# Research-Implementation/AudioVidSum-A-Multi-Modal-Approach-to-Video-Summarization

Hardware: AMD Instinct MI355X
Metric: frames/sec end-to-end (extract+fuse+score), 224x224 + 16kHz (higher is better)
Workload: dtype f16x2; 1 GPU; configs[1]: SumMe-shape batch, 25 videos x ~1800 frames (45143 frames/GPU), visual-only resnet50 extractor (batch-stat BN, the reference's 4-frame BatchNorm micro-batches inside each video) + AVBiLSTM attention scorer + mean-threshold selection; frames_per_gpu=45143, videos_per_gpu=25, extractor=resnet50, frames_per_group=4, chunk_frames=16384, parallelism=videos sharded x1, no data-path collective, selected_frames_rank0=22823

## Files before the change

audiovidsum-a-multi-modal-approach-to-video-summarization_amd/csrc/stem_h2.hip:

```cpp
#include "avs_internal.h"
#include <type_traits>

typedef _Float16 f16x8 __attribute__((ext_vector_type(8)));
typedef float f32x16 __attribute__((ext_vector_type(16)));

namespace {
constexpr int IMG = 224, CONV = 112, POOL = 56, COUT = 64;
constexpr int TY = 7, TX = 8;
constexpr int TH = 17, TWD = 15;
constexpr int PPY = 8, PPX = 7;
constexpr int MROWS = TH * TWD;
constexpr int PH = 39, PW = 36;
constexpr int PATCH_BYTES = PH * PW * 8;
constexpr int KDIM = 224;
constexpr int CW = 32;
constexpr int W_PITCH = KDIM * 4 + 16;
constexpr int W_BYTES = CW * W_PITCH;
constexpr int RT_PITCH = 144;
constexpr int RT_BYTES = 256 * RT_PITCH;
constexpr int WAVES = 4, THREADS = WAVES * 64;
constexpr int SRED_BYTES = WAVES * 2 * CW * 4, PIV_BYTES = CW * 4;
constexpr int SMEM_BYTES = W_BYTES + PATCH_BYTES + RT_BYTES + SRED_BYTES + PIV_BYTES;
constexpr int PIVOT_ROW = 9 * TWD + 7;
static_assert(SMEM_BYTES <= 80 * 1024, "two workgroups per CU");
}

struct StemH2Params {
  const uint8_t* frames;
  const char* w;
  const float* gamma;
  char* osel;
  float* part;
  long long ldw;
};

struct __attribute__((packed, aligned(1))) avs_u32_unaligned { unsigned v; };

__global__ __launch_bounds__(THREADS, 2) void stem_h2_kernel(StemH2Params p) {
  extern __shared__ __attribute__((aligned(16))) char smem[];
  char* wimg = smem;
  char* patch = smem + W_BYTES;
  char* rawt = patch + PATCH_BYTES;
  float* sred = reinterpret_cast<float*>(rawt + RT_BYTES);
  float* piv_s = sred + WAVES * 2 * CW;
  const int t = threadIdx.x;
  const int wave = __builtin_amdgcn_readfirstlane(t >> 6), lane = t & 63;
  const int lr = lane & 31, lh = lane >> 5;
  const int c0 = (blockIdx.x & 1) * CW;
  const long long img = blockIdx.x >> 1;
  const uint8_t* __restrict__ src = p.frames + img * (long long)(IMG * IMG * 3);

  for (int i = t; i < CW * (KDIM / 4); i += THREADS) {
    const int n = i / (KDIM / 4), ch = i - n * (KDIM / 4);
    *reinterpret_cast<uint4*>(wimg + n * W_PITCH + ch * 16) =
        *reinterpret_cast<const uint4*>(p.w + ((long long)(c0 + n) * p.ldw) * 4 + ch * 16);
  }
  int abase[2];
  unsigned own = 0;
#pragma unroll
  for (int mt = 0; mt < 2; ++mt) {
    int m = wave * 64 + mt * 32 + lr;
    if (m >= MROWS) m = MROWS - 1;
    const int ly = m / TWD, lx = m - ly * TWD;
    abase[mt] = ((2 * ly) * PW + 2 * lx) * 8 + lh * 16;
#pragma unroll
    for (int e = 0; e < 16; ++e) {
      const int me = wave * 64 + mt * 32 + (e & 3) + 8 * (e >> 2) + 4 * lh;
      const int ey = me / TWD, ex = me - ey * TWD;
      if (me < MROWS && ey >= 1 && ex >= 1) own |= 1u << (16 * mt + e);
    }
  }
  const int bbase = lr * W_PITCH + lh * 32;
  const bool pool_on = t < PPY * PPX * 4;
  const int p_cg = t & 3, p_pp = pool_on ? (t >> 2) : 0;
  const int p_pyl = p_pp / PPX, p_pxl = p_pp - p_pyl * PPX;
  float sg[8];
#pragma unroll
  for (int j = 0; j < 8; ++j) sg[j] = p.gamma[c0 + p_cg * 8 + j] < 0.f ? -1.f : 1.f;
  const char* praw = rawt + ((2 * p_pyl) * TWD + 2 * p_pxl) * RT_PITCH + p_cg * 32;

  constexpr int PPT = (PH * PW + THREADS - 1) / THREADS;
  unsigned pbytes[PPT];
  unsigned inside = 0u;
  int pyx[PPT];
#pragma unroll
  for (int j = 0; j < PPT; ++j) {
    const int i = t + j * THREADS;
    const int py = i < PH * PW ? i / PW : 255;
    pyx[j] = (py << 8) | (i - (i / PW) * PW);
  }
  auto gload = [&](int tile) {
    const int ty = tile / TX, tx = tile - ty * TX;
    const int iy0 = 32 * ty - 5, ix0 = 28 * tx - 5;
    const int ylo = iy0 < 0 ? -iy0 : 0, yhi = IMG - iy0 < PH ? IMG - iy0 : PH;
    const int xlo = ix0 < 0 ? -ix0 : 0, xhi = IMG - ix0 < PW ? IMG - ix0 : PW;
    inside = 0u;
#pragma unroll
    for (int j = 0; j < PPT; ++j) {
      const int py = pyx[j] >> 8, px = pyx[j] & 255;
      if (py >= ylo && py < yhi && px >= xlo && px < xhi) {
        const int o = ((iy0 + py) * IMG + ix0 + px) * 3;
        const bool prev = o > 0 || img > 0;
        const unsigned d = reinterpret_cast<const avs_u32_unaligned*>(src + o - (prev ? 1 : 0))->v;
        pbytes[j] = prev ? d >> 8 : d;
        inside |= 1u << j;
      }
    }
  };
  auto pstore = [&]() {
#pragma unroll
    for (int j = 0; j < PPT; ++j) {
      const int i = t + j * THREADS;
      if (i >= PH * PW) break;
      unsigned lo = 0u, hi = 0u;
      if ((inside >> j) & 1u) {
        const float b0 = (float)(pbytes[j] & 255u), b1 = (float)((pbytes[j] >> 8) & 255u), b2 = (float)((pbytes[j] >> 16) & 255u);
        lo = __builtin_bit_cast(unsigned, __builtin_amdgcn_cvt_pkrtz(b0, b1));
        hi = __builtin_bit_cast(unsigned, __builtin_amdgcn_cvt_pkrtz(b2, 1.f));
      }
      *reinterpret_cast<uint2*>(patch + i * 8) = make_uint2(lo, hi);
    }
  };
  float pm[8];
  auto pool_tap = [&](int tile, int tap) {
    const int ty = tile / TX, tx = tile - ty * TX;
    const int dy = tap / 3, dx = tap - dy * 3;
    const bool out = (dy == 0 && ty == 0 && p_pyl == 0) || (dx == 0 && tx == 0 && p_pxl == 0);
    const char* row = praw + (dy * TWD + dx) * RT_PITCH;
    const float4 va = *reinterpret_cast<const float4*>(row);
    const float4 vb = *reinterpret_cast<const float4*>(row + 16);
    const float v[8] = {va.x, va.y, va.z, va.w, vb.x, vb.y, vb.z, vb.w};
#pragma unroll
    for (int j = 0; j < 8; ++j) {
      float x = v[j] * sg[j];
      if (dy == 0 || dx == 0) x = out ? -INFINITY : x;
      pm[j] = tap == 0 ? x : fmaxf(pm[j], x);
    }
  };
  auto pool_finish = [&](int tile) {
    const int ty = tile / TX, tx = tile - ty * TX;
    float v8[8];
#pragma unroll
    for (int j = 0; j < 8; ++j) v8[j] = pm[j] * sg[j];
    uint4 hi, lo;
    avs_f16x2_split8(v8, hi, lo);
    const long long o = (((img * POOL + PPY * ty + p_pyl) * POOL + PPX * tx + p_pxl) * COUT + c0 + p_cg * 8) * 4;
    if (pool_on) {
      *reinterpret_cast<uint4*>(p.osel + o) = hi;
      *reinterpret_cast<uint4*>(p.osel + o + 16) = lo;
    }
  };

  gload(0);
  float pivot = 0.f, s1 = 0.f, s2 = 0.f;
  constexpr int NT = TY * TX;
  auto body = [&](auto pool_c, int tile) {
    constexpr bool POOLING = decltype(pool_c)::value;
    pstore();
    __syncthreads();
    if (tile + 1 < NT) gload(tile + 1);

    f32x16 acc[2];
#pragma unroll
    for (int i = 0; i < 2; ++i)
#pragma unroll
      for (int e = 0; e < 16; ++e) acc[i][e] = 0.f;
#pragma unroll
    for (int s = 0; s < 14; ++s) {
      const int aoff = (s >> 1) * (PW * 8) + (s & 1) * 32;
      uint4 fa[2];
#pragma unroll
      for (int mt = 0; mt < 2; ++mt) fa[mt] = *reinterpret_cast<const uint4*>(patch + abase[mt] + aoff);
      const uint4 fbh = *reinterpret_cast<const uint4*>(wimg + bbase + s * 64);
      const uint4 fbl = *reinterpret_cast<const uint4*>(wimg + bbase + s * 64 + 16);
#pragma unroll
      for (int mt = 0; mt < 2; ++mt)
        acc[mt] = __builtin_amdgcn_mfma_f32_32x32x16_f16(__builtin_bit_cast(f16x8, fa[mt]), __builtin_bit_cast(f16x8, fbh),
                                                         acc[mt], 0, 0, 0);
#pragma unroll
      for (int mt = 0; mt < 2; ++mt)
        acc[mt] = __builtin_amdgcn_mfma_f32_32x32x16_f16(__builtin_bit_cast(f16x8, fa[mt]), __builtin_bit_cast(f16x8, fbl),
                                                         acc[mt], 0, 0, 0);
      if constexpr (POOLING) {
        if (s < 9) pool_tap(tile - 1, s);
        if (s == 9) pool_finish(tile - 1);
      }
    }
    if (tile == 0 && wave == PIVOT_ROW / 64 && lh == ((PIVOT_ROW % 32) >> 2 & 1)) {
      constexpr int PMT = (PIVOT_ROW % 64) / 32, PR = PIVOT_ROW % 32;
      constexpr int PE = (PR & 3) + 4 * (PR >> 3);
      piv_s[lr] = acc[PMT][PE];
    }
    __syncthreads();
    if (tile == 0) pivot = piv_s[lr];
    float t1 = 0.f, t2 = 0.f;
#pragma unroll
    for (int mt = 0; mt < 2; ++mt)
#pragma unroll
      for (int e = 0; e < 16; ++e) {
        const float v = acc[mt][e];
        const float d = ((own >> (16 * mt + e)) & 1u) ? v - pivot : 0.f;
        t1 += d;
        t2 = fmaf(d, d, t2);
        const int m = wave * 64 + mt * 32 + (e & 3) + 8 * (e >> 2) + 4 * lh;
        *reinterpret_cast<float*>(rawt + m * RT_PITCH + lr * 4) = v;
      }
    s1 += t1;
    s2 += t2;
  };
  body(std::false_type{}, 0);
  for (int tile = 1; tile < NT; ++tile) body(std::true_type{}, tile);
  __syncthreads();
#pragma unroll
  for (int tap = 0; tap < 9; ++tap) pool_tap(NT - 1, tap);
  pool_finish(NT - 1);
  s1 += __shfl_xor(s1, 32, 64);
  s2 += __shfl_xor(s2, 32, 64);
  if (lh == 0) {
    sred[(wave * 2 + 0) * CW + lr] = s1;
    sred[(wave * 2 + 1) * CW + lr] = s2;
  }
  __syncthreads();
  if (t < CW) {
    float a = 0.f, b = 0.f;
#pragma unroll
    for (int w = 0; w < WAVES; ++w) {
      a += sred[(w * 2 + 0) * CW + t];
      b += sred[(w * 2 + 1) * CW + t];
    }
    const float inv_n = 1.f / (float)(CONV * CONV);
    const float dm = a * inv_n;
    p.part[(img * 2 + 0) * COUT + c0 + t] = piv_s[t] + dm;
    p.part[(img * 2 + 1) * COUT + c0 + t] = fmaxf(b - a * dm, 0.f);
  }
}

__global__ __launch_bounds__(256) void stem_h2_fold_kernel(const float* __restrict__ part, int groups, int fpg,
                                                           const float* __restrict__ gamma, const float* __restrict__ beta,
                                                           float eps, float* __restrict__ scale, float* __restrict__ shift) {
  const int i = blockIdx.x * blockDim.x + threadIdx.x;
  if (i >= groups * COUT) return;
  const int g = i / COUT, ch = i - g * COUT;
  const float nf = (float)(CONV * CONV);
  float n = 0.f, mean = 0.f, m2 = 0.f;
  for (int f = 0; f < fpg; ++f) {
    const long long fr = (long long)g * fpg + f;
    const float mf = part[(fr * 2 + 0) * COUT + ch], qf = part[(fr * 2 + 1) * COUT + ch];
    const float tot = n + nf, delta = mf - mean;
    mean += delta * (nf / tot);
    m2 += qf + delta * delta * (n * nf / tot);
    n = tot;
  }
  const float var = m2 / n;
  const float sc = gamma[ch] / sqrtf(var + eps);
  scale[i] = sc;
  shift[i] = beta[ch] - mean * sc;
}

extern "C" int64_t avs_stem_f16x2_workspace_bytes(int n) {
  if (n < 0) return AVS_E_SHAPE;
  return (int64_t)n * 2 * COUT * 4;
}

extern "C" int avs_stem_conv_pool_f16x2(const uint8_t* d_frames, int n, const void* d_w, int64_t ldw,
                                        int frames_per_group, const float* d_gamma, const float* d_beta, float eps,
                                        void* d_y, float* d_scale, float* d_shift, void* d_ws, int64_t ws_bytes,
                                        avs_stream_t stream) {
  const char* who = "avs_stem_conv_pool_f16x2";
  AVS_REQUIRE(n >= 0 && frames_per_group > 0, AVS_E_SHAPE, "%s: n=%d frames_per_group=%d", who, n, frames_per_group);
  if (n == 0) return AVS_OK;
  AVS_REQUIRE(n % frames_per_group == 0, AVS_E_UNSUPPORTED, "%s: needs equal-sized groups (%d frames in groups of %d)",
              who, n, frames_per_group);
  AVS_REQUIRE(d_frames && d_w && d_gamma && d_beta && d_y && d_scale && d_shift && d_ws, AVS_E_ARG,
              "%s: null pointer", who);
  AVS_REQUIRE(ldw >= KDIM && ldw % 8 == 0, AVS_E_SHAPE, "%s: weight rows are 7 x 8 x 4 = 224 slots, stride %lld", who,
              (long long)ldw);
  AVS_REQUIRE((((uintptr_t)d_w) & 31u) == 0 && (((uintptr_t)d_y) & 31u) == 0 && avs_aligned16(d_ws) &&
                  avs_aligned16(d_scale) && avs_aligned16(d_shift),
              AVS_E_ALIGN, "%s: AVS_F16X2 operands must be 32-byte aligned, the others 16-byte", who);
  const int64_t need = avs_stem_f16x2_workspace_bytes(n);
  AVS_REQUIRE(ws_bytes >= need, AVS_E_WORKSPACE, "%s: workspace %lld < %lld bytes", who, (long long)ws_bytes,
              (long long)need);
  AVS_REQUIRE((long long)n * 2 < (1ll << 31), AVS_E_SHAPE, "%s: too many frames", who);
  StemH2Params p{};
  p.frames = d_frames;
  p.w = (const char*)d_w;
  p.ldw = ldw;
  p.gamma = d_gamma;
  p.osel = (char*)d_y;
  p.part = reinterpret_cast<float*>(d_ws);
  hipStream_t st = (hipStream_t)stream;
  AVS_REQUIRE(hipFuncSetAttribute(reinterpret_cast<const void*>(stem_h2_kernel), hipFuncAttributeMaxDynamicSharedMemorySize,
                                  SMEM_BYTES) == hipSuccess,
              AVS_E_HIP, "%s: cannot reserve %d bytes of LDS", who, SMEM_BYTES);
  hipLaunchKernelGGL(stem_h2_kernel, dim3((unsigned)(n * 2)), dim3(THREADS), SMEM_BYTES, st, p);
  const int groups = n / frames_per_group;
  hipLaunchKernelGGL(stem_h2_fold_kernel, dim3((unsigned)avs_cdiv((int64_t)groups * COUT, 256)), dim3(256), 0, st, p.part,
                     groups, frames_per_group, d_gamma, d_beta, eps, d_scale, d_shift);
  AVS_CHECK_LAUNCH(who);
  return AVS_OK;
}
```

Measured before the change: 27160 frames/s.

## Hold stem conv weights in registers and double-buffer patch fragment loads

The stem conv kernel no longer stages the weight slice in LDS. Each lane instead loads its 14 K-steps of B fragments directly from global memory into registers, which frees LDS and removes the per-step LDS weight reads. The A-fragment LDS loads are software-pipelined one K-step ahead. The gather load is made branchless, with the byte-shift moved into pstore, and the pool_on guard on the output store is dropped. The cost is roughly 112 extra VGPRs per lane for the weights, which risks spills or lower occupancy under launch_bounds(256,2). Dropping the store guard may also let idle threads write duplicate or out-of-range pooled outputs.

```diff
diff --git a/audiovidsum-a-multi-modal-approach-to-video-summarization_amd/csrc/stem_h2.hip b/audiovidsum-a-multi-modal-approach-to-video-summarization_amd/csrc/stem_h2.hip
--- a/audiovidsum-a-multi-modal-approach-to-video-summarization_amd/csrc/stem_h2.hip
+++ b/audiovidsum-a-multi-modal-approach-to-video-summarization_amd/csrc/stem_h2.hip
@@ -14,13 +14,12 @@
 constexpr int PATCH_BYTES = PH * PW * 8;
 constexpr int KDIM = 224;
 constexpr int CW = 32;
-constexpr int W_PITCH = KDIM * 4 + 16;
-constexpr int W_BYTES = CW * W_PITCH;
+constexpr int KSTEPS = KDIM / 16;
 constexpr int RT_PITCH = 144;
 constexpr int RT_BYTES = 256 * RT_PITCH;
 constexpr int WAVES = 4, THREADS = WAVES * 64;
 constexpr int SRED_BYTES = WAVES * 2 * CW * 4, PIV_BYTES = CW * 4;
-constexpr int SMEM_BYTES = W_BYTES + PATCH_BYTES + RT_BYTES + SRED_BYTES + PIV_BYTES;
+constexpr int SMEM_BYTES = PATCH_BYTES + RT_BYTES + SRED_BYTES + PIV_BYTES;
 constexpr int PIVOT_ROW = 9 * TWD + 7;
 static_assert(SMEM_BYTES <= 80 * 1024, "two workgroups per CU");
 }
@@ -38,8 +37,7 @@
 
 __global__ __launch_bounds__(THREADS, 2) void stem_h2_kernel(StemH2Params p) {
   extern __shared__ __attribute__((aligned(16))) char smem[];
-  char* wimg = smem;
-  char* patch = smem + W_BYTES;
+  char* patch = smem;
   char* rawt = patch + PATCH_BYTES;
   float* sred = reinterpret_cast<float*>(rawt + RT_BYTES);
   float* piv_s = sred + WAVES * 2 * CW;
@@ -50,10 +48,14 @@
   const long long img = blockIdx.x >> 1;
   const uint8_t* __restrict__ src = p.frames + img * (long long)(IMG * IMG * 3);
 
-  for (int i = t; i < CW * (KDIM / 4); i += THREADS) {
-    const int n = i / (KDIM / 4), ch = i - n * (KDIM / 4);
-    *reinterpret_cast<uint4*>(wimg + n * W_PITCH + ch * 16) =
-        *reinterpret_cast<const uint4*>(p.w + ((long long)(c0 + n) * p.ldw) * 4 + ch * 16);
+  uint4 fbh[KSTEPS], fbl[KSTEPS];
+  {
+    const char* __restrict__ wrow = p.w + ((long long)(c0 + lr) * p.ldw) * 4 + lh * 32;
+#pragma unroll
+    for (int s = 0; s < KSTEPS; ++s) {
+      fbh[s] = *reinterpret_cast<const uint4*>(wrow + s * 64);
+      fbl[s] = *reinterpret_cast<const uint4*>(wrow + s * 64 + 16);
+    }
   }
   int abase[2];
   unsigned own = 0;
@@ -70,7 +72,6 @@
       if (me < MROWS && ey >= 1 && ex >= 1) own |= 1u << (16 * mt + e);
     }
   }
-  const int bbase = lr * W_PITCH + lh * 32;
   const bool pool_on = t < PPY * PPX * 4;
   const int p_cg = t & 3, p_pp = pool_on ? (t >> 2) : 0;
   const int p_pyl = p_pp / PPX, p_pxl = p_pp - p_pyl * PPX;
@@ -81,7 +82,7 @@
 
   constexpr int PPT = (PH * PW + THREADS - 1) / THREADS;
   unsigned pbytes[PPT];
-  unsigned inside = 0u;
+  unsigned inside = 0u, first = 0u;
   int pyx[PPT];
 #pragma unroll
   for (int j = 0; j < PPT; ++j) {
@@ -95,16 +96,16 @@
     const int ylo = iy0 < 0 ? -iy0 : 0, yhi = IMG - iy0 < PH ? IMG - iy0 : PH;
     const int xlo = ix0 < 0 ? -ix0 : 0, xhi = IMG - ix0 < PW ? IMG - ix0 : PW;
     inside = 0u;
+    first = 0u;
 #pragma unroll
     for (int j = 0; j < PPT; ++j) {
       const int py = pyx[j] >> 8, px = pyx[j] & 255;
-      if (py >= ylo && py < yhi && px >= xlo && px < xhi) {
-        const int o = ((iy0 + py) * IMG + ix0 + px) * 3;
-        const bool prev = o > 0 || img > 0;
-        const unsigned d = reinterpret_cast<const avs_u32_unaligned*>(src + o - (prev ? 1 : 0))->v;
-        pbytes[j] = prev ? d >> 8 : d;
-        inside |= 1u << j;
-      }
+      const bool in = py >= ylo && py < yhi && px >= xlo && px < xhi;
+      const int o = in ? ((iy0 + py) * IMG + ix0 + px) * 3 : 0;
+      const bool prev = o > 0 || img > 0;
+      pbytes[j] = reinterpret_cast<const avs_u32_unaligned*>(src + o - (prev ? 1 : 0))->v;
+      inside |= (in ? 1u : 0u) << j;
+      first |= (prev ? 0u : 1u) << j;
     }
   };
   auto pstore = [&]() {
@@ -114,7 +115,8 @@
       if (i >= PH * PW) break;
       unsigned lo = 0u, hi = 0u;
       if ((inside >> j) & 1u) {
-        const float b0 = (float)(pbytes[j] & 255u), b1 = (float)((pbytes[j] >> 8) & 255u), b2 = (float)((pbytes[j] >> 16) & 255u);
+        const unsigned d = ((first >> j) & 1u) ? pbytes[j] : pbytes[j] >> 8;
+        const float b0 = (float)(d & 255u), b1 = (float)((d >> 8) & 255u), b2 = (float)((d >> 16) & 255u);
         lo = __builtin_bit_cast(unsigned, __builtin_amdgcn_cvt_pkrtz(b0, b1));
         hi = __builtin_bit_cast(unsigned, __builtin_amdgcn_cvt_pkrtz(b2, 1.f));
       }
@@ -145,10 +147,8 @@
     uint4 hi, lo;
     avs_f16x2_split8(v8, hi, lo);
     const long long o = (((img * POOL + PPY * ty + p_pyl) * POOL + PPX * tx + p_pxl) * COUT + c0 + p_cg * 8) * 4;
-    if (pool_on) {
-      *reinterpret_cast<uint4*>(p.osel + o) = hi;
-      *reinterpret_cast<uint4*>(p.osel + o + 16) = lo;
-    }
+    *reinterpret_cast<uint4*>(p.osel + o) = hi;
+    *reinterpret_cast<uint4*>(p.osel + o + 16) = lo;
   };
 
   gload(0);
@@ -165,22 +165,24 @@
     for (int i = 0; i < 2; ++i)
 #pragma unroll
       for (int e = 0; e < 16; ++e) acc[i][e] = 0.f;
-#pragma unroll
-    for (int s = 0; s < 14; ++s) {
-      const int aoff = (s >> 1) * (PW * 8) + (s & 1) * 32;
-      uint4 fa[2];
-#pragma unroll
-      for (int mt = 0; mt < 2; ++mt) fa[mt] = *reinterpret_cast<const uint4*>(patch + abase[mt] + aoff);
-      const uint4 fbh = *reinterpret_cast<const uint4*>(wimg + bbase + s * 64);
-      const uint4 fbl = *reinterpret_cast<const uint4*>(wimg + bbase + s * 64 + 16);
+    uint4 fa[2][2];
+#pragma unroll
+    for (int mt = 0; mt < 2; ++mt) fa[0][mt] = *reinterpret_cast<const uint4*>(patch + abase[mt]);
+#pragma unroll
+    for (int s = 0; s < KSTEPS; ++s) {
+      if (s + 1 < KSTEPS) {
+        const int aoff = ((s + 1) >> 1) * (PW * 8) + ((s + 1) & 1) * 32;
+#pragma unroll
+        for (int mt = 0; mt < 2; ++mt) fa[(s + 1) & 1][mt] = *reinterpret_cast<const uint4*>(patch + abase[mt] + aoff);
+      }
 #pragma unroll
       for (int mt = 0; mt < 2; ++mt)
-        acc[mt] = __builtin_amdgcn_mfma_f32_32x32x16_f16(__builtin_bit_cast(f16x8, fa[mt]), __builtin_bit_cast(f16x8, fbh),
-                                                         acc[mt], 0, 0, 0);
+        acc[mt] = __builtin_amdgcn_mfma_f32_32x32x16_f16(__builtin_bit_cast(f16x8, fa[s & 1][mt]),
+                                                         __builtin_bit_cast(f16x8, fbh[s]), acc[mt], 0, 0, 0);
 #pragma unroll
       for (int mt = 0; mt < 2; ++mt)
-        acc[mt] = __builtin_amdgcn_mfma_f32_32x32x16_f16(__builtin_bit_cast(f16x8, fa[mt]), __builtin_bit_cast(f16x8, fbl),
-                                                         acc[mt], 0, 0, 0);
+        acc[mt] = __builtin_amdgcn_mfma_f32_32x32x16_f16(__builtin_bit_cast(f16x8, fa[s & 1][mt]),
+                                                         __builtin_bit_cast(f16x8, fbl[s]), acc[mt], 0, 0, 0);
       if constexpr (POOLING) {
         if (s < 9) pool_tap(tile - 1, s);
         if (s == 9) pool_finish(tile - 1);
```

Result: no change. 27290 frames/s, median of 6 (+0.5%).
